# vwxyzjn/cleanrl

Hardware: AMD Instinct MI355X
Metric: env-steps/sec (SPS) PPO Breakout num_envs=1024 @1/2/4/8 MI355X; GAE HBM GB/s (higher is better)
Workload: dtype f32

## Files before the change

cleanrl_amd/build.py:

```python
from __future__ import annotations

import os
import subprocess
import sys
from concurrent.futures import ThreadPoolExecutor

CSRC = os.path.join(os.path.dirname(os.path.abspath(__file__)), "csrc")
LIB = os.path.join(CSRC, "libmi355ppo.so")
SOURCES = ["api.hip", "gae.hip", "distributions.hip", "loss.hip", "obs.hip", "optim.hip", "conv.hip", "convw.hip", "conv1q.hip", "conv1p.hip", "gemmz.hip", "gemmg.hip", "gemmh.hip", "convr.hip", "convrb.hip", "convu.hip", "fcw.hip", "heads.hip", "mlp.hip", "synth_env.hip", "dpcomm.hip", "lstm.hip", "trxl_attn.hip", "impala.hip", "pqn.hip", "pqn_lstm.hip", "offpolicy.hip", "sac.hip", "dqn.hip", "dqn_atari.hip", "rainbow.hip", "rainbow_twins.hip", "sac_atari.hip", "sac_atari_twins.hip", "qdagger.hip", "rnd.hip", "ppg.hip", "ppg_twins.hip", "host_twins.hip"]
HEADERS = ["common.h", "catrow.h", "ppo_rows.h", "lstm_rows.h", "trxl_rows.h", "impala_rows.h", "pqn_rows.h", "pqn_lstm_rows.h", "offpolicy_rows.h", "offpolicy_wg.h", "qhead_wg.h", "sac_rows.h", "dqn_rows.h", "dqn_atari_rows.h", "rainbow_rows.h", "sac_atari_rows.h", "qdagger_rows.h", "rnd_rows.h", "ppg_rows.h", "bf16split.h", "f16split.h", "convr_geom.h", "convrb_geom.h", os.path.join("..", "..", "include", "mi355ppo.h")]
HIPCC = os.environ.get("HIPCC", "/opt/rocm/bin/hipcc")
FLAGS = ["--offload-arch=gfx950", "-O3", "-std=c++20", "-ffp-contract=off", "-fPIC", "-fvisibility=hidden", "-Wall", "-Wno-unused-function"]
EXTRA_FLAGS = {"conv.hip": ["-mllvm", "-pragma-unroll-threshold=1000000"], "gemmz.hip": ["-fno-slp-vectorize"], "gemmg.hip": ["-fno-slp-vectorize"], "gemmh.hip": ["-fno-slp-vectorize", "-mllvm", "-pragma-unroll-threshold=1000000"], "convr.hip": ["-fno-slp-vectorize", "-mllvm", "-pragma-unroll-threshold=1000000"], "convrb.hip": ["-fno-slp-vectorize", "-mllvm", "-pragma-unroll-threshold=1000000"], "convu.hip": ["-fno-slp-vectorize", "-mllvm", "-pragma-unroll-threshold=1000000"], "fcw.hip": ["-fno-slp-vectorize"], "convw.hip": ["-fno-slp-vectorize"], "lstm.hip": ["-fno-slp-vectorize"], "pqn_lstm.hip": ["-fno-slp-vectorize"]}


def _stale(target: str, deps: list[str]) -> bool:
    if not os.path.exists(target):
        return True
    t = os.path.getmtime(target)
    return any(os.path.getmtime(d) > t for d in deps)


def _run(cmd: list[str]) -> None:
    r = subprocess.run(cmd, cwd=CSRC, capture_output=True, text=True)
    if r.returncode != 0:
        raise RuntimeError("command failed: %s\n%s\n%s" % (" ".join(cmd), r.stdout, r.stderr))


def build(force: bool = False, verbose: bool = True) -> str:
    hdrs = [os.path.join(CSRC, h) for h in HEADERS]
    objs, jobs = [], []
    for src in SOURCES:
        obj = os.path.join(CSRC, src.replace(".hip", ".o"))
        objs.append(obj)
        if force or _stale(obj, [os.path.join(CSRC, src)] + hdrs):
            jobs.append([HIPCC] + FLAGS + EXTRA_FLAGS.get(src, []) + ["-c", src, "-o", obj])
    if jobs:
        if verbose:
            print(f"[cleanrl_amd.build] compiling {len(jobs)} HIP source(s) for gfx950", file=sys.stderr)
        with ThreadPoolExecutor(max_workers=min(len(jobs), os.cpu_count() or 1)) as ex:
            list(ex.map(_run, jobs))
    if force or jobs or _stale(LIB, objs):
        _run([HIPCC, "--offload-arch=gfx950", "-shared", "-o", LIB] + objs)
        if verbose:
            print(f"[cleanrl_amd.build] linked {LIB}", file=sys.stderr)
    return LIB


def build_tools(verbose: bool = True) -> str:
    root = os.path.dirname(os.path.dirname(CSRC))
    src = os.path.join(root, "tools", "conv_traffic.cpp")
    exe = os.path.join(root, "tools", "conv_traffic")
    if _stale(exe, [src, LIB, os.path.join(root, "include", "mi355ppo.h")]):
        _run([HIPCC, "--offload-arch=gfx950", "-O2", "-I" + os.path.join(root, "include"), src, "-o", exe, "-L" + CSRC,
              "-lmi355ppo", "-Wl,-rpath,$ORIGIN/../cleanrl_amd/csrc"])
        if verbose:
            print(f"[cleanrl_amd.build] built {exe}", file=sys.stderr)
    fsrc, fexe = os.path.join(root, "tools", "mfma_floor.cpp"), os.path.join(root, "tools", "mfma_floor")
    if os.path.exists(fsrc) and _stale(fexe, [fsrc]):
        _run([HIPCC, "--offload-arch=gfx950", "-O3", fsrc, "-o", fexe])
        if verbose:
            print(f"[cleanrl_amd.build] built {fexe}", file=sys.stderr)
    psrc, pexe = os.path.join(root, "tools", "hbm_probe.cpp"), os.path.join(root, "tools", "hbm_probe")
    if os.path.exists(psrc) and _stale(pexe, [psrc]):
        _run([HIPCC, "--offload-arch=gfx950", "-O3", psrc, "-o", pexe])
        if verbose:
            print(f"[cleanrl_amd.build] built {pexe}", file=sys.stderr)
    dsrc, dexe = os.path.join(root, "tools", "mfma_denorm.cpp"), os.path.join(root, "tools", "mfma_denorm")
    if os.path.exists(dsrc) and _stale(dexe, [dsrc]):
        _run([HIPCC, "--offload-arch=gfx950", "-O2", "-Wno-unused-result", dsrc, "-o", dexe])
        if verbose:
            print(f"[cleanrl_amd.build] built {dexe}", file=sys.stderr)
    return exe


if __name__ == "__main__":
    build(force="--force" in sys.argv)
    build_tools()
```

cleanrl_amd/csrc/common.h:

```cpp
#pragma once
#include <hip/hip_runtime.h>
#include <stdint.h>
#include <stdio.h>
#include <stdarg.h>
#include <stdlib.h>

#include "../../include/mi355ppo.h"

#define MI355_WAVE 64
#ifndef MI355_AUX_WGRAD_LD
#define MI355_AUX_WGRAD_LD 2
#endif
#ifndef MI355_AUX_STREAM_LD
#define MI355_AUX_STREAM_LD 0
#endif
#ifndef MI355_AUX_STREAM_ST
#define MI355_AUX_STREAM_ST 0
#endif
#define MI355_HD __host__ __device__ __forceinline__

namespace mi355ppo {

void set_error(const char* fmt, ...);

int conv1p_launch(const unsigned char* src, const int64_t* inds, const float* dz, float* part_w, float* part_b, int images, int grid,
                  hipStream_t s, const unsigned* dz_amax, float* partial_scale);
bool convw_applies(int64_t images, int layer, bool f16 = false);
int convw_parts(int64_t images, int layer);
int convw_launch(const float* src, const float* dz, float* part_w, float* part_b, int64_t images, int layer, int* nparts, hipStream_t s,
                 const unsigned* dz_amax = nullptr, const unsigned* src_amax = nullptr);

bool convr_on(long long images, long long min_images);
int convr_fwd3(const char* fn, const float* src, unsigned src_bytes, const void* pack, const float* bias, float* dst, unsigned dst_bytes, unsigned* bits,
               long long images, const unsigned* src_amax, unsigned* dst_amax, hipStream_t st);
int convr_fwd2(const char* fn, const float* src, unsigned src_bytes, const void* pack, const float* bias, float* dst, unsigned dst_bytes, unsigned* bits,
               long long images, const unsigned* src_amax, unsigned* dst_amax, hipStream_t st);
int convr_dgrad3(const char* fn, const float* dz, unsigned dz_bytes, const void* pack, const unsigned* bits, float* dsrc, unsigned dsrc_bytes,
                 long long images, const unsigned* dz_amax, unsigned* dsrc_amax, hipStream_t st);
int convr_dgrad2(const char* fn, const float* dz, unsigned dz_bytes, const void* pack, const unsigned* bits, float* dsrc, unsigned dsrc_bytes,
                 long long images, const unsigned* dz_amax, unsigned* dsrc_amax, hipStream_t st);
#ifndef MI355_RING_DMA
#define MI355_RING_DMA 1
#endif
#ifndef MI355_RB_MIN_IMAGES
#define MI355_RB_MIN_IMAGES 3072
#endif
bool convrb_takes(long long images);
int convrb_dgrad2(const char* fn, const float* dz, unsigned dz_bytes, const void* pack, const unsigned* bits, float* dsrc, unsigned dsrc_bytes,
                  long long images, const unsigned* dz_amax, unsigned* dsrc_amax, hipStream_t st);
int convu_max_parts();
bool convu_takes(int64_t images, int layer);
int convu_launch(const float* src, const float* dz, float* part_w, float* part_b, int64_t images, int layer, int* nparts, hipStream_t s,
                 const unsigned* dz_amax, const unsigned* src_amax);
int convu1_launch(const unsigned char* frames, const int64_t* inds, const float* dz, float* part_w, float* part_b, int64_t images, int* nparts,
                  hipStream_t s, const unsigned* dz_amax);
bool gemmg_on(long long rows, long long min_rows);
int gemmg_launch(const char* fn, int epi, const float* A, int lda, const void* pack, const float* bias, const unsigned* bits, float* C, int M, int N,
                 int K, const unsigned* a_amax, unsigned* c_amax, hipStream_t s);
bool gemmh_takes(int M, int N, int K, int lddz);
int gemmh_slabs();
int gemmh_launch(const float* dz, int lddz, const float* a, float* part, int M, int N, int K, const unsigned* dz_amax, const unsigned* a_amax, hipStream_t s);
int z_fc_raw_launch(const char* fn, const float* a, int lda, const void* pack, int M, int N, int K, void* ws, size_t ws_bytes, int* splits,
                    hipStream_t stream, const unsigned* a_amax = nullptr);

inline hipStream_t as_stream(void* s) { return reinterpret_cast<hipStream_t>(s); }

inline int bf16_term_pairs() {
    static const int n = [] {
        const char* e = getenv("MI355PPO_BF16_PAIRS");
        return (e && e[0] == '9') ? 9 : 6;
    }();
    return n;
}

inline bool kernel_switch(const char* name, long long size, long long default_min) {
    const char* e = getenv(name);
    if (!e || !e[0]) return size >= default_min;
    if (e[0] == '0' && !e[1]) return false;
    if (e[0] == 'm' && e[1] == 'i' && e[2] == 'n' && e[3] == ':') return size >= atoll(e + 4);
    return size >= default_min;
}

inline bool aligned(const void* p, size_t a) { return (reinterpret_cast<uintptr_t>(p) % a) == 0; }

inline int check_launch(const char* what) {
    hipError_t e = hipGetLastError();
    if (e != hipSuccess) {
        set_error("%s: %s", what, hipGetErrorString(e));
        return MI355PPO_EHIP;
    }
    return MI355PPO_OK;
}

#define MI355_REQUIRE(cond, code, ...)          \
    do {                                        \
        if (!(cond)) {                          \
            ::mi355ppo::set_error(__VA_ARGS__); \
            return (code);                      \
        }                                       \
    } while (0)

#ifdef __HIPCC__

MI355_HD uint32_t mulhi_u32(uint32_t a, uint32_t b) {
#if defined(__HIP_DEVICE_COMPILE__)
    return __umulhi(a, b);
#else
    return (uint32_t)(((uint64_t)a * (uint64_t)b) >> 32);
#endif
}

struct Philox {
    uint32_t k0, k1;
    MI355_HD Philox(uint64_t seed) : k0((uint32_t)seed), k1((uint32_t)(seed >> 32)) {}
    MI355_HD uint4 operator()(uint64_t ctr_lo, uint64_t ctr_hi) const {
        uint32_t c0 = (uint32_t)ctr_lo, c1 = (uint32_t)(ctr_lo >> 32), c2 = (uint32_t)ctr_hi, c3 = (uint32_t)(ctr_hi >> 32);
        uint32_t a = k0, b = k1;
#pragma unroll
        for (int r = 0; r < 10; ++r) {
            const uint32_t hi0 = mulhi_u32(0xD2511F53u, c0), lo0 = 0xD2511F53u * c0;
            const uint32_t hi1 = mulhi_u32(0xCD9E8D57u, c2), lo1 = 0xCD9E8D57u * c2;
            const uint32_t n0 = hi1 ^ c1 ^ a, n1 = lo1, n2 = hi0 ^ c3 ^ b, n3 = lo0;
            c0 = n0; c1 = n1; c2 = n2; c3 = n3;
            a += 0x9E3779B9u; b += 0xBB67AE85u;
        }
        return make_uint4(c0, c1, c2, c3);
    }
};

MI355_HD float u32_to_unit_open(uint32_t x) {
    return ((float)(x >> 9) + 0.5f) * (1.0f / 8388608.0f);
}


__device__ __forceinline__ float wave_sum(float v) {
#pragma unroll
    for (int off = 32; off > 0; off >>= 1) v += __shfl_xor(v, off, MI355_WAVE);
    return v;
}
__device__ __forceinline__ double wave_sum(double v) {
#pragma unroll
    for (int off = 32; off > 0; off >>= 1) v += __shfl_xor(v, off, MI355_WAVE);
    return v;
}

template <int NWAVES>
__device__ __forceinline__ double block_sum(double v, double* lds) {
    v = wave_sum(v);
    const int lane = threadIdx.x & 63, wave = threadIdx.x >> 6;
    if (lane == 0) lds[wave] = v;
    __syncthreads();
    double r = 0.0;
    if (threadIdx.x == 0) {
#pragma unroll
        for (int w = 0; w < NWAVES; ++w) r += lds[w];
    }
    __syncthreads();
    return r;
}

#endif
}
```

cleanrl_amd/csrc/gemmz.hip:

```cpp
#include "common.h"
#include "conv1q_pack.h"
#include "bf16split.h"
#include "f16split.h"
#include <type_traits>

#pragma clang fp contract(off)

namespace mi355ppo {

typedef float z_f32x16 __attribute__((ext_vector_type(16)));

__device__ __forceinline__ int z_writelane(int w, unsigned x, int l) {
    asm("s_nop 1\n\tv_writelane_b32 %0, %1, %2" : "+v"(w) : "s"(x), "i"(l));
    return w;
}

enum { Z_BIAS_RELU = 0, Z_MASK = 1, Z_MASK_CLS4 = 2, Z_MASKB = 3, Z_MASKB_CLS4 = 4, Z_BIAS_RELU_BITS = 5, Z_RAW = 6 };

__device__ __forceinline__ float z_keep_where(float x, unsigned lo, unsigned hi) {
    const unsigned long long m = ((unsigned long long)hi << 32) | lo;
    float r;
    asm("s_nop 1\n\tv_cndmask_b32_e64 %0, 0, %1, %2" : "=v"(r) : "v"(x), "s"(m));
    return r;
}
// ... 954 lines not shown
}

__global__ __launch_bounds__(256) void zsplit_reduce_kernel(const float4* __restrict__ part, int splits, size_t slab4, const float* __restrict__ bias,
                                                            int n4, float4* __restrict__ h, size_t total4) {
    const size_t i = (size_t)blockIdx.x * 256 + threadIdx.x;
    if (i >= total4) return;
    float4 acc = part[i];
    for (int z = 1; z < splits; ++z) {
        const float4 p = part[(size_t)z * slab4 + i];
        acc.x += p.x; acc.y += p.y; acc.z += p.z; acc.w += p.w;
    }
    const float* const b = bias + 4 * (i % (size_t)n4);
    acc.x += b[0]; acc.y += b[1]; acc.z += b[2]; acc.w += b[3];
    h[i] = make_float4(acc.x > 0.0f ? acc.x : 0.0f, acc.y > 0.0f ? acc.y : 0.0f, acc.z > 0.0f ? acc.z : 0.0f, acc.w > 0.0f ? acc.w : 0.0f);
}

static int zsplit_steps_per(int M, int N, int K) {
    const long long tiles = (long long)((M + 63) / 64) * ((N + 63) / 64);
    const int total = K / 16;
    int target = 2 * M;
    if (target < 256) target = 256;
    if (target > 1024) target = 1024;
    long long want = (target + tiles - 1) / tiles;
    if (want < 1) want = 1;
    int per = (int)((total + want - 1) / want);
    if (per < 4) per = 4;
    if (per > total) per = total;
    return per;
}

extern "C" MI355PPO_API size_t mi355ppo_fc_fwd_workspace_bytes(int M, int N, int K) {
    constexpr int below = 8192;
    if (M <= 0 || N <= 0 || K <= 0 || K % 16 || M >= below) return 0;
    const int per = zsplit_steps_per(M, N, K), splits = (K / 16 + per - 1) / per;
    return splits > 1 ? (size_t)splits * (size_t)M * (size_t)N * sizeof(float) : 0;
}

static bool fc_g_takes(int M, int N, int K, bool dgrad) {
    return M > 0 && N > 0 && N % 32 == 0 && K >= 128 && K % 64 == 0 && gemmg_on(M, dgrad ? 1024 : 16384);
}
extern "C" MI355PPO_API int mi355ppo_fc_packed_kernel_f16x2(int M, int N, int K, int dgrad) { return fc_g_takes(M, N, K, dgrad != 0) ? 'G' : 'Z'; }

static int fc_fwd_impl(const char* fn, const float* a, int lda, const void* pack, const float* bias, float* h, int M, int N, int K,
                       const unsigned* a_amax, unsigned* h_amax, void* stream) {
    int rc = zgemm_check(fn, a, pack, h, M, N, K, lda, N);
    if (rc) return rc;
    MI355_REQUIRE(bias && aligned(bias, 4), MI355PPO_EINVAL, "%s: bias missing or misaligned", fn);
    ZArgs za = zargs(a, (long long)M * lda * 4, lda, pack, bias, nullptr, h, (long long)M * N * 4, N, M, N, K);
    za.a_amax = a_amax; za.c_amax = h_amax;
    if (a_amax && fc_g_takes(M, N, K, false)) {
        rc = gemmg_launch(fn, 0, a, lda, pack, bias, nullptr, h, M, N, K, a_amax, h_amax, as_stream(stream));
        if (rc <= 0) return rc;
    }
    if (M < 16384) return z_launch<ZRowsLinear, 2, 2, 4, Z_BIAS_RELU, true, 2>(za, as_stream(stream), fn);
    return z_launch<ZRowsLinear, 2, 4, 4, Z_BIAS_RELU, true>(za, as_stream(stream), fn);
}

extern "C" MI355PPO_API int mi355ppo_fc_fwd_relu_packed_f32(const float* a, int lda, const void* pack, const float* bias, float* h,
                                                            int M, int N, int K, void* stream) {
    return fc_fwd_impl("mi355ppo_fc_fwd_relu_packed_f32", a, lda, pack, bias, h, M, N, K, nullptr, nullptr, stream);
}

static int fc_fwd_ws_impl(const char* fn, const float* a, int lda, const void* pack, const float* bias, float* h, int M, int N, int K, void* ws,
                          size_t ws_bytes, const unsigned* a_amax, unsigned* h_amax, void* stream) {
    const size_t need = mi355ppo_fc_fwd_workspace_bytes(M, N, K);
    if (need == 0 || !ws || N % 4) return fc_fwd_impl(fn, a, lda, pack, bias, h, M, N, K, a_amax, h_amax, stream);
    MI355_REQUIRE(!h_amax, MI355PPO_EINVAL, "%s: the K-split forward (M=%d) does not record h's maximum (no consumer splits h: pass null)", fn, M);
    int rc = zgemm_check(fn, a, pack, h, M, N, K, lda, N);
    if (rc) return rc;
    MI355_REQUIRE(bias && aligned(bias, 4) && aligned(h, 16) && aligned(ws, 16), MI355PPO_EINVAL, "%s: bias missing, or h / workspace not 16-byte aligned", fn);
    MI355_REQUIRE(ws_bytes >= need, MI355PPO_EINVAL, "%s: workspace of %zu bytes, %zu needed (mi355ppo_fc_fwd_workspace_bytes)", fn, ws_bytes, need);
    ZArgs za = zargs(a, (long long)M * lda * 4, lda, pack, bias, nullptr, static_cast<float*>(ws), (long long)M * N * 4, N, M, N, K);
    za.a_amax = a_amax;
    za.steps_per = zsplit_steps_per(M, N, K);
    const int splits = (K / 16 + za.steps_per - 1) / za.steps_per;
    rc = z_launch<ZRowsLinear, 2, 2, 4, Z_RAW, true, 2>(za, as_stream(stream), fn);
    if (rc) return rc;
    const size_t total4 = (size_t)M * N / 4;
    hipLaunchKernelGGL(zsplit_reduce_kernel, dim3((unsigned)((total4 + 255) / 256)), dim3(256), 0, as_stream(stream),
                       static_cast<const float4*>(ws), splits, total4, bias, N / 4, reinterpret_cast<float4*>(h), total4);
    return check_launch(fn);
}

extern "C" MI355PPO_API int mi355ppo_fc_fwd_relu_packed_ws_f32(const float* a, int lda, const void* pack, const float* bias, float* h,
                                                               int M, int N, int K, void* ws, size_t ws_bytes, void* stream) {
    return fc_fwd_ws_impl("mi355ppo_fc_fwd_relu_packed_ws_f32", a, lda, pack, bias, h, M, N, K, ws, ws_bytes, nullptr, nullptr, stream);
}

namespace mi355ppo {
int z_fc_raw_launch(const char* fn, const float* a, int lda, const void* pack, int M, int N, int K, void* ws, size_t ws_bytes, int* splits,
                    hipStream_t stream, const unsigned* a_amax) {
    const size_t need = mi355ppo_fc_fwd_workspace_bytes(M, N, K);
    MI355_REQUIRE(need > 0 && N % 4 == 0, MI355PPO_EINVAL, "%s: M=%d rows need no K split (use the unfused entry points from 8,192 rows on)", fn, M);
    int rc = zgemm_check(fn, a, pack, static_cast<const float*>(ws), M, N, K, lda, N);
    if (rc) return rc;
    MI355_REQUIRE(ws && aligned(ws, 16) && ws_bytes >= need, MI355PPO_EWORKSPACE, "%s: workspace of %zu bytes, %zu needed (mi355ppo_fc_fwd_workspace_bytes)",
                  fn, ws ? ws_bytes : (size_t)0, need);
    ZArgs za = zargs(a, (long long)M * lda * 4, lda, pack, nullptr, nullptr, static_cast<float*>(ws), (long long)M * N * 4, N, M, N, K);
    za.a_amax = a_amax;
    za.steps_per = zsplit_steps_per(M, N, K);
    *splits = (K / 16 + za.steps_per - 1) / za.steps_per;
    return z_launch<ZRowsLinear, 2, 2, 4, Z_RAW, true, 2>(za, stream, fn);
}
}

static int fc_dgrad_impl(const char* fn, const float* dz, int lddz, const void* pack, const float* act_in, const unsigned* bits, float* da,
                         int M, int N, int K, void* stream, const unsigned* dz_amax = nullptr, unsigned* da_amax = nullptr) {
    int rc = zgemm_check(fn, dz, pack, da, M, N, K, lddz, N);
    if (rc) return rc;
    ZArgs za = zargs(dz, (long long)M * lddz * 4, lddz, pack, nullptr, act_in, da, (long long)M * N * 4, N, M, N, K);
    za.a_amax = dz_amax; za.c_amax = da_amax;
    za.super_rows = 4;
    if (bits) {
        MI355_REQUIRE(N % 32 == 0 && aligned(bits, 4) && aligned(da, 128), MI355PPO_EINVAL, "%s: bit masks need N %% 32 == 0 (N=%d) and da on a 128-byte boundary", fn, N);
        za.bits_in = bits;
        if (dz_amax && fc_g_takes(M, N, K, true)) {
            rc = gemmg_launch(fn, 1, dz, lddz, pack, nullptr, bits, da, M, N, K, dz_amax, da_amax, as_stream(stream));
            if (rc <= 0) return rc;
        }
        return z_launch<ZRowsLinear, 2, 4, 4, Z_MASKB, false>(za, as_stream(stream), fn);
    }
    MI355_REQUIRE(act_in && aligned(act_in, 4) && act_in != da, MI355PPO_EINVAL, "%s: act_in missing, misaligned or aliased with da", fn);
    return z_launch<ZRowsLinear, 2, 4, 4, Z_MASK, false>(za, as_stream(stream), fn);
}

extern "C" MI355PPO_API int mi355ppo_fc_dgrad_mask_packed_f32(const float* dz, int lddz, const void* pack, const float* act_in, float* da,
                                                              int M, int N, int K, void* stream) {
    return fc_dgrad_impl("mi355ppo_fc_dgrad_mask_packed_f32", dz, lddz, pack, act_in, nullptr, da, M, N, K, stream);
}

extern "C" MI355PPO_API int mi355ppo_fc_dgrad_maskbits_packed_f32(const float* dz, int lddz, const void* pack, const uint32_t* mask_bits,
                                                                  float* da, int M, int N, int K, void* stream) {
    const char* fn = "mi355ppo_fc_dgrad_maskbits_packed_f32";
    MI355_REQUIRE(mask_bits, MI355PPO_EINVAL, "%s: null pointer", fn);
    return fc_dgrad_impl(fn, dz, lddz, pack, nullptr, mask_bits, da, M, N, K, stream);
}

static bool conv_r_takes(long long images, int layer, bool dgrad) {
    return convr_on(images, dgrad && layer == 2 ? 512 : 1);
}

static int conv_fwd_packed_impl(const char* fn, const float* src, const void* pack, const float* bias, float* dst, unsigned* bits,
                                int64_t images, int layer, void* stream, const unsigned* src_amax = nullptr, unsigned* dst_amax = nullptr) {
    MI355_REQUIRE(src && pack && bias && dst, MI355PPO_EINVAL, "%s: null pointer", fn);
    MI355_REQUIRE(layer == 2 || layer == 3, MI355PPO_EINVAL, "%s: layer=%d must be 2 or 3", fn, layer);
    MI355_REQUIRE(images > 0, MI355PPO_EINVAL, "%s: images=%lld must be positive", fn, (long long)images);
    MI355_REQUIRE(aligned(src, 16) && aligned(pack, 16) && aligned(dst, 128) && aligned(bias, 4) && aligned(bits, 4), MI355PPO_EALIGN,
                  "%s: src / pack must be 16-byte aligned, dst 128-byte aligned", fn);
    const long long srcb = (long long)images * (layer == 2 ? 20 * 20 * 32 : 9 * 9 * 64) * 4;
    MI355_REQUIRE(srcb < (1LL << 32) - 8192, MI355PPO_EINVAL, "%s: the source (%lld bytes) must stay below 4 GiB (32-bit buffer offsets)", fn, srcb);
    hipStream_t st = as_stream(stream);
    const bool small = !bits && images < 768;
    if (layer == 2) {
        if (src_amax && conv_r_takes(images, 2, false))
            return convr_fwd2(fn, src, (unsigned)srcb, pack, bias, dst, (unsigned)((long long)images * 81 * 64 * 4), bits, images, src_amax, dst_amax, st);
        ZArgs za = zargs(src, srcb, 0, pack, bias, nullptr, dst, (long long)images * 81 * 64 * 4, 64, (long long)images * 81, 64, ZConv2::K);
        za.bits_out = bits;
        za.a_amax = src_amax; za.c_amax = dst_amax;
        if (small) return z_launch<ZConv2, 1, 2, 4, Z_BIAS_RELU, false, 2>(za, st, fn);
        if (bits) return z_blds(images) ? z_launch<ZConv2, 2, 2, 4, Z_BIAS_RELU_BITS, false, 2, true>(za, st, fn) : z_launch<ZConv2, 2, 2, 4, Z_BIAS_RELU_BITS, false, 2>(za, st, fn);
        return z_blds(images) ? z_launch<ZConv2, 2, 2, 4, Z_BIAS_RELU, false, 2, true>(za, st, fn) : z_launch<ZConv2, 2, 2, 4, Z_BIAS_RELU, false, 2>(za, st, fn);
    }
    if (src_amax && conv_r_takes(images, 3, false))
        return convr_fwd3(fn, src, (unsigned)srcb, pack, bias, dst, (unsigned)((long long)images * 49 * 64 * 4), bits, images, src_amax, dst_amax, st);
    ZArgs za = zargs(src, srcb, 0, pack, bias, nullptr, dst, (long long)images * 49 * 64 * 4, 64, (long long)images * 49, 64, ZConv3::K);
    za.bits_out = bits;
    za.a_amax = src_amax; za.c_amax = dst_amax;
    if (small) return z_launch<ZConv3, 1, 2, 4, Z_BIAS_RELU, false, 2>(za, st, fn);
    if (bits) return z_blds(images) ? z_launch<ZConv3, 2, 2, 4, Z_BIAS_RELU_BITS, false, 2, true>(za, st, fn) : z_launch<ZConv3, 2, 2, 4, Z_BIAS_RELU_BITS, false, 2>(za, st, fn);
    return z_blds(images) ? z_launch<ZConv3, 2, 2, 4, Z_BIAS_RELU, false, 2, true>(za, st, fn) : z_launch<ZConv3, 2, 2, 4, Z_BIAS_RELU, false, 2>(za, st, fn);
}

extern "C" MI355PPO_API int mi355ppo_cnn_conv_fwd_packed_f32(const float* src, const void* pack, const float* bias, float* dst,
                                                             int64_t images, int layer, void* stream) {
    return conv_fwd_packed_impl("mi355ppo_cnn_conv_fwd_packed_f32", src, pack, bias, dst, nullptr, images, layer, stream);
}

extern "C" MI355PPO_API int mi355ppo_cnn_conv_fwd_packed_bits_f32(const float* src, const void* pack, const float* bias, float* dst,
                                                                  uint32_t* mask_bits, int64_t images, int layer, void* stream) {
    const char* fn = "mi355ppo_cnn_conv_fwd_packed_bits_f32";
    MI355_REQUIRE(mask_bits, MI355PPO_EINVAL, "%s: null pointer", fn);
    return conv_fwd_packed_impl(fn, src, pack, bias, dst, mask_bits, images, layer, stream);
}

static int conv_dgrad_packed_impl(const char* fn, const float* dz, const void* pack, const float* act_in, const unsigned* bits, float* dsrc,
                                  int64_t images, int layer, void* stream, const unsigned* dz_amax = nullptr, unsigned* dsrc_amax = nullptr) {
    MI355_REQUIRE(dz && pack && (act_in || bits) && dsrc, MI355PPO_EINVAL, "%s: null pointer", fn);
    MI355_REQUIRE(layer == 2 || layer == 3, MI355PPO_EINVAL, "%s: layer=%d must be 2 or 3", fn, layer);
    MI355_REQUIRE(images > 0, MI355PPO_EINVAL, "%s: images=%lld must be positive", fn, (long long)images);
    MI355_REQUIRE(aligned(dz, 16) && aligned(pack, 16) && aligned(dsrc, 128) && aligned(act_in, 16) && aligned(bits, 4), MI355PPO_EALIGN,
                  "%s: dz / pack / act_in must be 16-byte aligned, dsrc 128-byte aligned", fn);
    MI355_REQUIRE(act_in != dsrc, MI355PPO_EINVAL, "%s: act_in must not alias dsrc", fn);
    const long long srcb = (long long)images * (layer == 2 ? 9 * 9 * 64 : 7 * 7 * 64) * 4;
    const long long dstb = (long long)images * (layer == 2 ? 20 * 20 * 32 : 9 * 9 * 64) * 4;
    MI355_REQUIRE(srcb < (1LL << 32) - 8192 && dstb < (1LL << 32) - 8192, MI355PPO_EINVAL,
                  "%s: dz (%lld bytes) and dsrc (%lld bytes) must stay below 4 GiB (32-bit buffer offsets)", fn, srcb, dstb);
    hipStream_t st = as_stream(stream);
    if (layer == 3) {
        if (dz_amax && bits && conv_r_takes(images, 3, true)) return convr_dgrad3(fn, dz, (unsigned)srcb, pack, bits, dsrc, (unsigned)dstb, images, dz_amax, dsrc_amax, st);
        ZArgs za = zargs(dz, srcb, 0, pack, nullptr, act_in, dsrc, (long long)images * 81 * 64 * 4, 64, (long long)images * 81, 64, ZDgrad3::K, images);
        za.bits_in = bits;
        za.a_amax = dz_amax; za.c_amax = dsrc_amax;
        if (bits) return z_blds(images) ? z_launch<ZDgrad3, 2, 2, 4, Z_MASKB, false, 2, true>(za, st, fn) : z_launch<ZDgrad3, 2, 2, 4, Z_MASKB, false, 2>(za, st, fn);
        return z_blds(images) ? z_launch<ZDgrad3, 2, 2, 4, Z_MASK, false, 2, true>(za, st, fn) : z_launch<ZDgrad3, 2, 2, 4, Z_MASK, false, 2>(za, st, fn);
    }
    if (dz_amax && bits && conv_r_takes(images, 2, true)) return convr_dgrad2(fn, dz, (unsigned)srcb, pack, bits, dsrc, (unsigned)dstb, images, dz_amax, dsrc_amax, st);
    ZArgs za = zargs(dz, srcb, 0, pack, nullptr, act_in, dsrc, (long long)images * 400 * 32 * 4, 0, (long long)images * 100, 128, ZDgrad2::K, images);
    za.bits_in = bits;
    za.a_amax = dz_amax; za.c_amax = dsrc_amax;
    if (bits) return z_blds(images) ? z_launch<ZDgrad2, 2, 2, 4, Z_MASKB_CLS4, false, 2, true>(za, st, fn) : z_launch<ZDgrad2, 2, 2, 4, Z_MASKB_CLS4, false, 2>(za, st, fn);
    return z_blds(images) ? z_launch<ZDgrad2, 2, 2, 4, Z_MASK_CLS4, false, 2, true>(za, st, fn) : z_launch<ZDgrad2, 2, 2, 4, Z_MASK_CLS4, false, 2>(za, st, fn);
}

extern "C" MI355PPO_API int mi355ppo_cnn_conv_dgrad_packed_f32(const float* dz, const void* pack, const float* act_in, float* dsrc,
                                                               int64_t images, int layer, void* stream) {
    const char* fn = "mi355ppo_cnn_conv_dgrad_packed_f32";
    MI355_REQUIRE(act_in, MI355PPO_EINVAL, "%s: null pointer", fn);
    return conv_dgrad_packed_impl(fn, dz, pack, act_in, nullptr, dsrc, images, layer, stream);
}

extern "C" MI355PPO_API int mi355ppo_cnn_conv_dgrad_packed_bits_f32(const float* dz, const void* pack, const uint32_t* mask_bits, float* dsrc,
                                                                    int64_t images, int layer, void* stream) {
    const char* fn = "mi355ppo_cnn_conv_dgrad_packed_bits_f32";
    MI355_REQUIRE(mask_bits, MI355PPO_EINVAL, "%s: null pointer", fn);
    return conv_dgrad_packed_impl(fn, dz, pack, nullptr, mask_bits, dsrc, images, layer, stream);
}

extern "C" MI355PPO_API int mi355ppo_cnn_conv_packed_kernel_f16x2(int64_t images, int layer, int dgrad) {
    if (!(images > 0 && (layer == 2 || layer == 3) && conv_r_takes(images, layer, dgrad != 0))) return 'Z';
    return (layer == 2 && dgrad != 0 && convrb_takes(images)) ? 'B' : 'R';
}

extern "C" MI355PPO_API size_t mi355ppo_fc_pack_f16x2_bytes(int N, int K) {
    if (N <= 0 || K <= 0 || K % 16) return 0;
    return (size_t)kF16PackHeader + (size_t)(K / 16) * (size_t)((N + 31) / 32) * 2048;
}

extern "C" MI355PPO_API int mi355ppo_absmax_f32(const float* x, int64_t n, uint32_t* amax, void* stream) {
    const char* fn = "mi355ppo_absmax_f32";
    MI355_REQUIRE(x && amax, MI355PPO_EINVAL, "%s: null pointer", fn);
    MI355_REQUIRE(n > 0, MI355PPO_EINVAL, "%s: n=%lld must be positive", fn, (long long)n);
    MI355_REQUIRE(aligned(x, 4) && aligned(amax, 64), MI355PPO_EALIGN, "%s: the amax record must be 64-byte aligned", fn);
    ZAbsmax3 m;
    m.x[0] = x; m.n[0] = n; m.x[1] = m.x[2] = x; m.n[1] = m.n[2] = 0;
    long long blocks = (n / 4 + 255) / 256;
    if (blocks < 1) blocks = 1;
    if (blocks > 2048) blocks = 2048;
    hipLaunchKernelGGL(zabsmax_kernel, dim3((unsigned)blocks), dim3(256), 0, as_stream(stream), m, amax, (int)blocks);
    return check_launch(fn);
}

extern "C" MI355PPO_API int mi355ppo_fc_pack_f16x2_f32(const float* B, int ldb, int N, int K, const uint32_t* b_amax, void* pack, void* stream) {
    const char* fn = "mi355ppo_fc_pack_f16x2_f32";
    MI355_REQUIRE(B && pack && b_amax, MI355PPO_EINVAL, "%s: null pointer", fn);
    MI355_REQUIRE(N > 0 && K > 0 && K % 16 == 0 && ldb >= K, MI355PPO_EINVAL, "%s: N=%d K=%d ldb=%d (K a positive multiple of 16, ldb >= K)", fn, N, K, ldb);
    MI355_REQUIRE(aligned(B, 4) && aligned(pack, 16) && aligned(b_amax, 64), MI355PPO_EALIGN, "%s: misaligned pointer (pack: 16 bytes, record: 64)", fn);
    const long long total = (long long)(K / 16) * ((N + 31) / 32) * 512;
    hipLaunchKernelGGL(zpack_h_kernel, dim3((unsigned)((total + 255) / 256)), dim3(256), 0, as_stream(stream), B, ldb, N, K, b_amax,
                       static_cast<unsigned char*>(pack));
    return check_launch(fn);
}

extern "C" MI355PPO_API int mi355ppo_fc_fwd_relu_packed_f16x2_f32(const float* a, int lda, const void* pack, const float* bias, float* h, int M,
                                                                  int N, int K, void* ws, size_t ws_bytes, const uint32_t* a_amax,
                                                                  uint32_t* h_amax, void* stream) {
    const char* fn = "mi355ppo_fc_fwd_relu_packed_f16x2_f32";
    MI355_REQUIRE(a_amax && aligned(a_amax, 64) && aligned(h_amax, 64), MI355PPO_EINVAL, "%s: a's amax record missing, or a record not 64-byte aligned", fn);
    return fc_fwd_ws_impl(fn, a, lda, pack, bias, h, M, N, K, ws, ws_bytes, a_amax, h_amax, stream);
}

extern "C" MI355PPO_API int mi355ppo_fc_dgrad_packed_f16x2_f32(const float* dz, int lddz, const void* pack, const float* act_in,
                                                               const uint32_t* mask_bits, float* da, int M, int N, int K, const uint32_t* dz_amax,
                                                               uint32_t* da_amax, void* stream) {
    const char* fn = "mi355ppo_fc_dgrad_packed_f16x2_f32";
    MI355_REQUIRE(dz_amax && aligned(dz_amax, 64) && aligned(da_amax, 64), MI355PPO_EINVAL, "%s: dz's amax record missing, or a record not 64-byte aligned", fn);
    MI355_REQUIRE(act_in || mask_bits, MI355PPO_EINVAL, "%s: neither act_in nor mask_bits", fn);
    return fc_dgrad_impl(fn, dz, lddz, pack, mask_bits ? nullptr : act_in, mask_bits, da, M, N, K, stream, dz_amax, da_amax);
}

extern "C" MI355PPO_API int mi355ppo_cnn_conv_fwd_packed_f16x2_f32(const float* src, const void* pack, const float* bias, float* dst,
                                                                   uint32_t* mask_bits, int64_t images, int layer, const uint32_t* src_amax,
                                                                   uint32_t* dst_amax, void* stream) {
    const char* fn = "mi355ppo_cnn_conv_fwd_packed_f16x2_f32";
    MI355_REQUIRE(src_amax && aligned(src_amax, 64) && aligned(dst_amax, 64), MI355PPO_EINVAL, "%s: src's amax record missing, or a record not 64-byte aligned", fn);
    return conv_fwd_packed_impl(fn, src, pack, bias, dst, mask_bits, images, layer, stream, src_amax, dst_amax);
}

extern "C" MI355PPO_API int mi355ppo_cnn_conv_dgrad_packed_f16x2_f32(const float* dz, const void* pack, const float* act_in,
                                                                     const uint32_t* mask_bits, float* dsrc, int64_t images, int layer,
                                                                     const uint32_t* dz_amax, uint32_t* dsrc_amax, void* stream) {
    const char* fn = "mi355ppo_cnn_conv_dgrad_packed_f16x2_f32";
    MI355_REQUIRE(dz_amax && aligned(dz_amax, 64) && aligned(dsrc_amax, 64), MI355PPO_EINVAL, "%s: dz's amax record missing, or a record not 64-byte aligned", fn);
    return conv_dgrad_packed_impl(fn, dz, pack, mask_bits ? nullptr : act_in, mask_bits, dsrc, images, layer, stream, dz_amax, dsrc_amax);
}
```

Baseline: 1.339 million.

## Add persistent stride-class conv2 forward kernel with pipelined f16 weight ring

Adds a new persistent forward kernel for conv layer 2 (20x20x32 -> 9x9x64, 4x4 stride 2). It decomposes the input into four stride-parity classes staged in LDS as split-f16 hi/lo records, and streams weights through a double-buffered DMA ring while the next group's activations are prefetched. The aim is to overlap global loads with MFMA work and cut redundant im2col-style traffic on the existing convr path. The cost is a large amount of hand-scheduled code with waitcnt/barrier logic that could be fragile. It is selected by default for batches of at least 512 images when the amax path is in use.

```diff
diff --git a/cleanrl_amd/build.py b/cleanrl_amd/build.py
--- a/cleanrl_amd/build.py
+++ b/cleanrl_amd/build.py
@@ -7,11 +7,11 @@
 
 CSRC = os.path.join(os.path.dirname(os.path.abspath(__file__)), "csrc")
 LIB = os.path.join(CSRC, "libmi355ppo.so")
-SOURCES = ["api.hip", "gae.hip", "distributions.hip", "loss.hip", "obs.hip", "optim.hip", "conv.hip", "convw.hip", "conv1q.hip", "conv1p.hip", "gemmz.hip", "gemmg.hip", "gemmh.hip", "convr.hip", "convrb.hip", "convu.hip", "fcw.hip", "heads.hip", "mlp.hip", "synth_env.hip", "dpcomm.hip", "lstm.hip", "trxl_attn.hip", "impala.hip", "pqn.hip", "pqn_lstm.hip", "offpolicy.hip", "sac.hip", "dqn.hip", "dqn_atari.hip", "rainbow.hip", "rainbow_twins.hip", "sac_atari.hip", "sac_atari_twins.hip", "qdagger.hip", "rnd.hip", "ppg.hip", "ppg_twins.hip", "host_twins.hip"]
-HEADERS = ["common.h", "catrow.h", "ppo_rows.h", "lstm_rows.h", "trxl_rows.h", "impala_rows.h", "pqn_rows.h", "pqn_lstm_rows.h", "offpolicy_rows.h", "offpolicy_wg.h", "qhead_wg.h", "sac_rows.h", "dqn_rows.h", "dqn_atari_rows.h", "rainbow_rows.h", "sac_atari_rows.h", "qdagger_rows.h", "rnd_rows.h", "ppg_rows.h", "bf16split.h", "f16split.h", "convr_geom.h", "convrb_geom.h", os.path.join("..", "..", "include", "mi355ppo.h")]
+SOURCES = ["api.hip", "gae.hip", "distributions.hip", "loss.hip", "obs.hip", "optim.hip", "conv.hip", "convw.hip", "conv1q.hip", "conv1p.hip", "gemmz.hip", "gemmg.hip", "gemmh.hip", "convr.hip", "convrb.hip", "convrs.hip", "convu.hip", "fcw.hip", "heads.hip", "mlp.hip", "synth_env.hip", "dpcomm.hip", "lstm.hip", "trxl_attn.hip", "impala.hip", "pqn.hip", "pqn_lstm.hip", "offpolicy.hip", "sac.hip", "dqn.hip", "dqn_atari.hip", "rainbow.hip", "rainbow_twins.hip", "sac_atari.hip", "sac_atari_twins.hip", "qdagger.hip", "rnd.hip", "ppg.hip", "ppg_twins.hip", "host_twins.hip"]
+HEADERS = ["common.h", "catrow.h", "ppo_rows.h", "lstm_rows.h", "trxl_rows.h", "impala_rows.h", "pqn_rows.h", "pqn_lstm_rows.h", "offpolicy_rows.h", "offpolicy_wg.h", "qhead_wg.h", "sac_rows.h", "dqn_rows.h", "dqn_atari_rows.h", "rainbow_rows.h", "sac_atari_rows.h", "qdagger_rows.h", "rnd_rows.h", "ppg_rows.h", "bf16split.h", "f16split.h", "convr_geom.h", "convrb_geom.h", "convrs_geom.h", os.path.join("..", "..", "include", "mi355ppo.h")]
 HIPCC = os.environ.get("HIPCC", "/opt/rocm/bin/hipcc")
 FLAGS = ["--offload-arch=gfx950", "-O3", "-std=c++20", "-ffp-contract=off", "-fPIC", "-fvisibility=hidden", "-Wall", "-Wno-unused-function"]
-EXTRA_FLAGS = {"conv.hip": ["-mllvm", "-pragma-unroll-threshold=1000000"], "gemmz.hip": ["-fno-slp-vectorize"], "gemmg.hip": ["-fno-slp-vectorize"], "gemmh.hip": ["-fno-slp-vectorize", "-mllvm", "-pragma-unroll-threshold=1000000"], "convr.hip": ["-fno-slp-vectorize", "-mllvm", "-pragma-unroll-threshold=1000000"], "convrb.hip": ["-fno-slp-vectorize", "-mllvm", "-pragma-unroll-threshold=1000000"], "convu.hip": ["-fno-slp-vectorize", "-mllvm", "-pragma-unroll-threshold=1000000"], "fcw.hip": ["-fno-slp-vectorize"], "convw.hip": ["-fno-slp-vectorize"], "lstm.hip": ["-fno-slp-vectorize"], "pqn_lstm.hip": ["-fno-slp-vectorize"]}
+EXTRA_FLAGS = {"conv.hip": ["-mllvm", "-pragma-unroll-threshold=1000000"], "gemmz.hip": ["-fno-slp-vectorize"], "gemmg.hip": ["-fno-slp-vectorize"], "gemmh.hip": ["-fno-slp-vectorize", "-mllvm", "-pragma-unroll-threshold=1000000"], "convr.hip": ["-fno-slp-vectorize", "-mllvm", "-pragma-unroll-threshold=1000000"], "convrb.hip": ["-fno-slp-vectorize", "-mllvm", "-pragma-unroll-threshold=1000000"], "convrs.hip": ["-fno-slp-vectorize", "-mllvm", "-pragma-unroll-threshold=1000000"], "convu.hip": ["-fno-slp-vectorize", "-mllvm", "-pragma-unroll-threshold=1000000"], "fcw.hip": ["-fno-slp-vectorize"], "convw.hip": ["-fno-slp-vectorize"], "lstm.hip": ["-fno-slp-vectorize"], "pqn_lstm.hip": ["-fno-slp-vectorize"]}
 
 
 def _stale(target: str, deps: list[str]) -> bool:
diff --git a/cleanrl_amd/csrc/common.h b/cleanrl_amd/csrc/common.h
--- a/cleanrl_amd/csrc/common.h
+++ b/cleanrl_amd/csrc/common.h
@@ -48,6 +48,12 @@
 bool convrb_takes(long long images);
 int convrb_dgrad2(const char* fn, const float* dz, unsigned dz_bytes, const void* pack, const unsigned* bits, float* dsrc, unsigned dsrc_bytes,
                   long long images, const unsigned* dz_amax, unsigned* dsrc_amax, hipStream_t st);
+#ifndef MI355_RS_MIN_IMAGES
+#define MI355_RS_MIN_IMAGES 512
+#endif
+bool convrs_takes(long long images);
+int convrs_fwd2(const char* fn, const float* src, unsigned src_bytes, const void* pack, const float* bias, float* dst, unsigned dst_bytes, unsigned* bits,
+                long long images, const unsigned* src_amax, unsigned* dst_amax, hipStream_t st);
 int convu_max_parts();
 bool convu_takes(int64_t images, int layer);
 int convu_launch(const float* src, const float* dz, float* part_w, float* part_b, int64_t images, int layer, int* nparts, hipStream_t s,
diff --git a/cleanrl_amd/csrc/convrs.hip b/cleanrl_amd/csrc/convrs.hip
--- /dev/null
+++ b/cleanrl_amd/csrc/convrs.hip
@@ -0,0 +1,267 @@
+#include "common.h"
+#include "f16split.h"
+#include "convrs_geom.h"
+
+#pragma clang fp contract(off)
+
+namespace mi355ppo {
+
+typedef float rs_f32x16 __attribute__((ext_vector_type(16)));
+
+constexpr unsigned kRSOob = 0xFFFFF000u;
+constexpr int kRSRsrcWord3 = 0x00020000;
+constexpr int kRSWaitVm0 = 0x0F70;
+
+__device__ __forceinline__ int rs_writelane(int w, unsigned x, int l) {
+    asm("s_nop 1\n\tv_writelane_b32 %0, %1, %2" : "+v"(w) : "s"(x), "i"(l));
+    return w;
+}
+
+__device__ __forceinline__ void rs_dma16(__amdgpu_buffer_rsrc_t rsrc, unsigned char* dst, unsigned voff, int soff) {
+    __builtin_amdgcn_raw_ptr_buffer_load_lds(rsrc, (__attribute__((address_space(3))) void*)dst, 16, voff, soff, 0, 0);
+}
+
+__device__ __forceinline__ void rs_put16(unsigned addr, unsigned long long hi, unsigned long long lo) {
+    asm volatile("ds_write2_b64 %0, %1, %2 offset1:8" : : "v"(addr), "v"(hi), "v"(lo) : "memory");
+}
+
+struct RSArgs {
+    const float* A;
+    unsigned a_bytes;
+    const unsigned char* pack;
+    const float* bias;
+    unsigned* bits_out;
+    float* C;
+    unsigned c_bytes;
+    long long images;
+    int groups;
+    const unsigned* a_amax;
+    unsigned* c_amax;
+};
+
+constexpr int rs_dma_younger(int slot) {
+    using RG = RSGeom;
+    int n = 0;
+    for (int r = 0; r < RG::NI; ++r) {
+        const int w = RG::round_step(r), lo = (slot * RG::SS) % RG::PSTEPS;
+        n += (w >= lo && w < lo + RG::SS - 1) ? 1 : 0;
+    }
+    return n;
+}
+
+template <bool BITS>
+__global__ __launch_bounds__(RSGeom::THREADS) __attribute__((amdgpu_waves_per_eu(2, 2))) void rs_kernel(RSArgs a) {
+    using RG = RSGeom;
+    constexpr int NT = RG::NT, NW = RG::NW, NI = RG::NI, THREADS = RG::THREADS, SS = RG::SS, NSLOT = RG::KSTEPS / SS, PSTEPS = RG::PSTEPS;
+    constexpr int kPieces = SS * NT * 2;
+    constexpr int kShare = kPieces / NW;
+    static_assert(kPieces % NW == 0 && NSLOT % 2 == 0, "whole pieces per wave; the next group's slot 0 goes to buffer 0 while the last slot is read from buffer 1");
+    __shared__ __attribute__((aligned(16))) unsigned char lds[RG::LDSB];
+    unsigned char* const ring = lds + RG::ABYTES;
+    const int tid = threadIdx.x, lane = tid & 63, wave = __builtin_amdgcn_readfirstlane(tid >> 6);
+    const int li = lane & 31, lh = lane >> 5;
+
+    const int ea = f16_scale_exp(amax_load(a.a_amax, lane));
+    const int eb = f16_scale_exp(*reinterpret_cast<const unsigned*>(a.pack));
+    const float sa = f16_pow2(ea), un = f16_unscale(ea, eb);
+
+    constexpr RRowTable<RG> table{};
+    auto row_pixel = [&](int slot, int& gi, int& gy, int& gx) __attribute__((always_inline)) {
+        const int rc = table.src[slot];
+        gi = rc / RG::OP;
+        const int pp = rc - gi * RG::OP;
+        gy = pp / RG::OW; gx = pp - gy * RG::OW;
+    };
+    constexpr unsigned kGroupC = RG::G * RG::OP * 32 * NT * 4;
+    static_assert(kGroupC < 65536, "two row offsets per register");
+    const unsigned char* win;
+    unsigned roff[8], rword;
+    {
+        int gi, gy, gx;
+        row_pixel(wave * 32 + li, gi, gy, gx);
+        win = lds + (gi * RG::IP + RG::pidx(gy, gx)) * RG::PIX + 16 * lh;
+        rword = (unsigned)((gi * RG::OP + gy * RG::OW + gx) * (32 * NT)) * 4u;
+#pragma unroll
+        for (int e = 0; e < 16; ++e) {
+            row_pixel(wave * 32 + (e & 3) + 8 * (e >> 2) + 4 * lh, gi, gy, gx);
+            const unsigned o = (unsigned)((gi * RG::OP + gy * RG::OW + gx) * (32 * NT)) * 4u + 4u * (unsigned)li;
+            roff[e >> 1] = (e & 1) ? (roff[e >> 1] | (o << 16)) : o;
+        }
+    }
+    const unsigned char* const ring_r = ring + 16 * lane;
+
+    unsigned usrc[NI], udst[NI];
+#pragma unroll
+    for (int r = 0; r < NI; ++r) {
+        const int u = r * THREADS + tid;
+        const int c4 = u % RG::UPP, j = (u / RG::UPP) % RG::CW, i = (u / (RG::UPP * RG::CW)) % RG::CH, img = u / (RG::UPP * RG::CW * RG::CH);
+        const bool ok = u < RG::CUNITS;
+        usrc[r] = ok ? (unsigned)(img * RG::IMG_SRC + (2 * i * RG::IW + 2 * j) * (RG::IC * 4) + c4 * 16) : kRSOob;
+        udst[r] = ok ? (unsigned)((img * RG::IP + i * RG::RP + j) * RG::PIX + c4 * 8) : (unsigned)(RG::SPARE * RG::PIX + c4 * 8);
+    }
+    auto rsrc_a_of = [&](int g) __attribute__((always_inline)) {
+        const bool ok = g < a.groups;
+        const unsigned gb = (unsigned)g * (unsigned)RG::GROUP_SRC;
+        return __builtin_amdgcn_make_buffer_rsrc(reinterpret_cast<unsigned char*>(const_cast<float*>(a.A)) + (ok ? gb : 0u), 0, ok ? (int)(a.a_bytes - gb) : 0, kRSRsrcWord3);
+    };
+    const unsigned lds_base = (unsigned)(uintptr_t)(__attribute__((address_space(3))) unsigned char*)lds;
+    static_assert(RG::LO == 64, "rs_put16: the lo half one ds_write2_b64 stride (8 x 8 bytes) behind the hi half");
+    s_u32x4 pre[NI];
+    auto get = [&](const __amdgpu_buffer_rsrc_t ra, int cls, int r) __attribute__((always_inline)) {
+        pre[r] = __builtin_bit_cast(s_u32x4, __builtin_amdgcn_raw_buffer_load_b128(ra, usrc[r] + (unsigned)(((cls >> 1) * RG::IW + (cls & 1)) * (RG::IC * 4)), 0, MI355_AUX_STREAM_LD));
+    };
+    auto put = [&](int buf, int r) __attribute__((always_inline)) {
+        unsigned hi[2], lo[2];
+        f16_split4(pre[r], sa, hi, lo);
+        rs_put16(lds_base + (unsigned)(buf * RG::BUFB) + udst[r], ((unsigned long long)hi[1] << 32) | hi[0], ((unsigned long long)lo[1] << 32) | lo[0]);
+    };
+
+    auto rsrc_c_of = [&](unsigned gbase) __attribute__((always_inline)) {
+        return __builtin_amdgcn_make_buffer_rsrc(reinterpret_cast<unsigned char*>(a.C) + gbase, 0, (int)(a.c_bytes - gbase), kRSRsrcWord3);
+    };
+    const __amdgpu_buffer_rsrc_t rsrc_b = __builtin_amdgcn_make_buffer_rsrc(BITS ? a.bits_out : nullptr, 0, BITS ? (int)(a.c_bytes >> 5) : 0, kRSRsrcWord3);
+    float bj[NT];
+#pragma unroll
+    for (int j = 0; j < NT; ++j) bj[j] = a.bias[32 * j + li];
+    float cmax = 0.0f;
+
+    const __amdgpu_buffer_rsrc_t rsrc_p = __builtin_amdgcn_make_buffer_rsrc(const_cast<unsigned char*>(a.pack), 0, kF16PackHeader + RG::KSTEPS * RG::STEPB, kRSRsrcWord3);
+    auto dma_slot = [&](int slot) __attribute__((always_inline)) {
+#pragma unroll
+        for (int u = 0; u < kShare; ++u) {
+            const int x = wave * kShare + u, h = x / (NT * 2), jt = x - h * (NT * 2);
+            rs_dma16(rsrc_p, ring + (slot & 1) * RG::SLOTB + x * 1024, 16u * (unsigned)lane, kF16PackHeader + r_kstep<RG>(SS * (slot % NSLOT) + h) * RG::STEPB + jt * 1024);
+        }
+    };
+    auto dma_wait = [&](int slot) __attribute__((always_inline)) {
+        const int n = rs_dma_younger(slot);
+#define RS_VMCNT_CASE(k) if (n == k) asm volatile("s_waitcnt vmcnt(" #k ")" ::: "memory");
+        RS_VMCNT_CASE(0) RS_VMCNT_CASE(1) RS_VMCNT_CASE(2) RS_VMCNT_CASE(3) RS_VMCNT_CASE(4)
+#undef RS_VMCNT_CASE
+        static_assert(RG::NI <= 5, "at most NI - 1 rounds behind a slot's pieces");
+    };
+    auto ring_barrier = [&]() __attribute__((always_inline)) {
+        asm volatile("s_waitcnt lgkmcnt(0)" ::: "memory");
+        __builtin_amdgcn_s_barrier();
+    };
+
+    rs_f32x16 acc[NT];
+    int wv = 0;
+    s_u32x4 pa[2][2], wb[2][NT][2];
+    auto read_a = [&](int par, int v) __attribute__((always_inline)) {
+        const int off = (rs_class(v) & 1) * RG::BUFB + rs_tapoff(r_kstep<RG>(v));
+        pa[par][0] = *reinterpret_cast<const s_u32x4*>(win + off);
+        pa[par][1] = *reinterpret_cast<const s_u32x4*>(win + off + RG::LO);
+    };
+    auto read_b = [&](int par, int v) __attribute__((always_inline)) {
+        const int buf = (v / SS) & 1, h = v % SS;
+#pragma unroll
+        for (int j = 0; j < NT; ++j)
+#pragma unroll
+            for (int t = 0; t < 2; ++t) wb[par][j][t] = *reinterpret_cast<const s_u32x4*>(ring_r + buf * RG::SLOTB + ((h * NT + j) * 2 + t) * 1024);
+    };
+    auto epi_elem = [&](int j, int e, unsigned gbase, const __amdgpu_buffer_rsrc_t rc) __attribute__((always_inline)) {
+        asm volatile("" : "+v"(roff[e >> 1]));
+        const unsigned rpk = roff[e >> 1];
+        const unsigned ro = ((e & 1) ? rpk >> 16 : rpk & 0xffffu) + (unsigned)(128 * j);
+        float v = __builtin_fmaf(acc[j][e], un, bj[j]);
+        v = v < 0.0f ? 0.0f : v;
+        cmax = __builtin_fmaxf(cmax, __builtin_fabsf(v));
+        __builtin_amdgcn_raw_buffer_store_b32(__float_as_uint(v), rc, ro, 0, MI355_AUX_STREAM_ST);
+        if constexpr (BITS) {
+            if (e == 0) wv = 0;
+            const unsigned long long bal = __builtin_amdgcn_ballot_w64(v > 0.0f);
+            wv = rs_writelane(wv, (unsigned)bal, (e & 3) + 8 * (e >> 2));
+            wv = rs_writelane(wv, (unsigned)(bal >> 32), (e & 3) + 8 * (e >> 2) + 4);
+            if (e == 15) __builtin_amdgcn_raw_buffer_store_b32((unsigned)wv, rsrc_b, lh == 0 ? (gbase + rword + (unsigned)(128 * j)) >> 5 : kRSOob, 0, 0);
+        }
+    };
+    static_assert(RG::round_step(NI - 1) < PSTEPS - 1, "a class is written before the barrier at its phase's last step");
+    auto group = [&](int grp) __attribute__((always_inline)) {
+        const unsigned gbase = (unsigned)grp * kGroupC;
+        const __amdgpu_buffer_rsrc_t ra_cur = rsrc_a_of(grp), ra_next = rsrc_a_of(grp + (int)gridDim.x);
+        ring_barrier();
+        read_a(0, 0);
+        read_b(0, 0);
+#pragma unroll
+        for (int v = 0; v < RG::KSTEPS; ++v) {
+            const int q = v & 1, slot = v / SS, h = v % SS, g = v / PSTEPS, w = v % PSTEPS;
+            if (h == SS - 1) dma_wait(slot);
+            if (v + 1 < RG::KSTEPS) {
+                if (h == SS - 1) ring_barrier();
+                read_b(q ^ 1, v + 1);
+                read_a(q ^ 1, v + 1);
+            }
+            if (h == 0) {
+                dma_slot(slot + 1);
+                __builtin_amdgcn_sched_barrier(0);
+            }
+#pragma unroll
+            for (int r = 0; r < NI; ++r)
+                if (w == RG::round_step(r)) {
+                    put((g + 1) & 1, r);
+                    get(g + 2 < RG::PHASES ? ra_cur : ra_next, (g + 2) % RG::PHASES, r);
+                }
+            __builtin_amdgcn_sched_barrier(0);
+#pragma unroll
+            for (int pi = 0; pi < 3; ++pi)
+#pragma unroll
+                for (int j = 0; j < NT; ++j) {
+                    if (v == 0 && pi == 0) {
+#pragma unroll
+                        for (int e = 0; e < 16; ++e) acc[j][e] = 0.0f;
+                    }
+                    acc[j] = __builtin_amdgcn_mfma_f32_32x32x16_f16(__builtin_bit_cast(s_f16x8, pa[q][pi == 2 ? 1 : 0]),
+                                                                    __builtin_bit_cast(s_f16x8, wb[q][j][pi == 1 ? 1 : 0]), acc[j], 0, 0, 0);
+                }
+            __builtin_amdgcn_sched_barrier(0);
+        }
+        const __amdgpu_buffer_rsrc_t rc = rsrc_c_of(gbase);
+#pragma unroll
+        for (int j = 0; j < NT; ++j)
+#pragma unroll
+            for (int e = 0; e < 16; ++e) epi_elem(j, e, gbase, rc);
+    };
+
+    int grp = blockIdx.x;
+    if (grp < a.groups) {
+        const __amdgpu_buffer_rsrc_t ra = rsrc_a_of(grp);
+#pragma unroll
+        for (int r = 0; r < NI; ++r) get(ra, 0, r);
+        dma_slot(0);
+        __builtin_amdgcn_s_waitcnt(kRSWaitVm0);
+#pragma unroll
+        for (int r = 0; r < NI; ++r) {
+            put(0, r);
+            get(ra, 1, r);
+        }
+        __builtin_amdgcn_s_waitcnt(kRSWaitVm0);
+    }
+    for (; grp < a.groups; grp += gridDim.x) group(grp);
+    if (a.c_amax) amax_commit(a.c_amax, __float_as_uint(cmax), blockIdx.x * NW + (unsigned)wave, lane);
+}
+
+bool convrs_takes(long long images) { return kernel_switch("MI355PPO_CONV_RS", images, MI355_RS_MIN_IMAGES); }
+
+int convrs_fwd2(const char* fn, const float* src, unsigned src_bytes, const void* pack, const float* bias, float* dst, unsigned dst_bytes, unsigned* bits,
+                long long images, const unsigned* src_amax, unsigned* dst_amax, hipStream_t st) {
+    RSArgs a{};
+    a.A = src; a.a_bytes = src_bytes; a.pack = static_cast<const unsigned char*>(pack); a.bias = bias; a.bits_out = bits; a.C = dst; a.c_bytes = dst_bytes;
+    a.images = images; a.a_amax = src_amax; a.c_amax = dst_amax;
+    a.groups = (int)((images + RSGeom::G - 1) / RSGeom::G);
+    static int cus = 0;
+    if (cus == 0) {
+        int dev = 0, n = 0;
+        if (hipGetDevice(&dev) != hipSuccess || hipDeviceGetAttribute(&n, hipDeviceAttributeMultiprocessorCount, dev) != hipSuccess || n <= 0) {
+            (void)hipGetLastError();
+            n = 256;
+        }
+        cus = n;
+    }
+    const int grid = a.groups < cus ? a.groups : cus;
+    if (bits) hipLaunchKernelGGL(rs_kernel<true>, dim3((unsigned)grid), dim3(RSGeom::THREADS), 0, st, a);
+    else hipLaunchKernelGGL(rs_kernel<false>, dim3((unsigned)grid), dim3(RSGeom::THREADS), 0, st, a);
+    return check_launch(fn);
+}
+
+}
diff --git a/cleanrl_amd/csrc/convrs_geom.h b/cleanrl_amd/csrc/convrs_geom.h
--- /dev/null
+++ b/cleanrl_amd/csrc/convrs_geom.h
@@ -0,0 +1,43 @@
+#pragma once
+
+#include "convr_geom.h"
+
+namespace mi355ppo {
+
+struct RSGeom {
+    static constexpr int IH = 20, IW = 20, IC = 32, KH = 4, KW = 4, S = 1, OH = 9, OW = 9, NT = 2, G = 3, NW = 8, MT = 1, ORDER = 2, SS = 4, WGS = 1;
+    static constexpr int NTW = NT, RW = NW;
+    static constexpr int PIX = 4 * IC + 16, LO = 2 * IC, C16 = IC / 16, UPP = IC / 4;
+    static constexpr int CH = IH / 2, CW = IW / 2;
+    static constexpr int RP = 10, IP = 101, IPIX = IP;
+    static constexpr int SPARE = CH * RP;
+    static constexpr int OP = OH * OW, ROWS = G * OP, SLOTS = 32 * MT * NW;
+    static constexpr int KSTEPS = KH * KW * C16, SPR = KW * C16, PHASES = 4, PSTEPS = KSTEPS / PHASES;
+    static constexpr int BUFB = G * IP * PIX, ABYTES = 2 * BUFB;
+    static constexpr int STEPB = NT * 2048, SLOTB = SS * STEPB;
+    static constexpr int LDSB = ABYTES + 2 * SLOTB;
+    static constexpr int THREADS = 64 * NW;
+    static constexpr int CUNITS = G * CH * CW * UPP, NI = (CUNITS + THREADS - 1) / THREADS;
+    static constexpr int IMG_SRC = IH * IW * IC * 4, GROUP_SRC = G * IMG_SRC;
+    static constexpr int pidx(int y, int x) { return y * RP + x; }
+    static constexpr int unit_src(int cls, int u) {
+        const int c4 = u % UPP, j = (u / UPP) % CW, i = (u / (UPP * CW)) % CH, img = u / (UPP * CW * CH);
+        return img * IMG_SRC + ((2 * i + (cls >> 1)) * IW + 2 * j + (cls & 1)) * (IC * 4) + c4 * 16;
+    }
+    static constexpr int unit_dst(int u) {
+        const int c4 = u % UPP, j = (u / UPP) % CW, i = (u / (UPP * CW)) % CH, img = u / (UPP * CW * CH);
+        return (img * IP + i * RP + j) * PIX + c4 * 8;
+    }
+    static constexpr int round_step(int r) { return r < 3 ? r : r + 1; }
+    static_assert((PIX / 16) % 2 == 1 && KSTEPS % (PHASES * SS) == 0 && PSTEPS == 2 * SS && ROWS <= SLOTS && NI == 5, "odd record pitch; whole ring slots per phase");
+    static_assert((G - 1) * IP + (CH - 1) * RP + CW <= G * IP && RP >= CW && IP >= CH * RP && SPARE < IP && (OH - 1 + 1) * RP + OW - 1 + 1 < SPARE, "class records inside the buffer");
+    static_assert(LDSB <= 160 * 1024, "LDS");
+};
+
+R_GEOM_FN int rs_class(int v) { return v / RSGeom::PSTEPS; }
+R_GEOM_FN int rs_tapoff(int ks) {
+    const int ty = ks / RSGeom::SPR, us = ks - ty * RSGeom::SPR, tx = us / RSGeom::C16, chunk = us - tx * RSGeom::C16;
+    return ((ty >> 1) * RSGeom::RP + (tx >> 1)) * RSGeom::PIX + chunk * 32;
+}
+
+}
diff --git a/cleanrl_amd/csrc/gemmz.hip b/cleanrl_amd/csrc/gemmz.hip
--- a/cleanrl_amd/csrc/gemmz.hip
+++ b/cleanrl_amd/csrc/gemmz.hip
@@ -1130,8 +1130,10 @@
     hipStream_t st = as_stream(stream);
     const bool small = !bits && images < 768;
     if (layer == 2) {
-        if (src_amax && conv_r_takes(images, 2, false))
+        if (src_amax && conv_r_takes(images, 2, false)) {
+            if (convrs_takes(images)) return convrs_fwd2(fn, src, (unsigned)srcb, pack, bias, dst, (unsigned)((long long)images * 81 * 64 * 4), bits, images, src_amax, dst_amax, st);
             return convr_fwd2(fn, src, (unsigned)srcb, pack, bias, dst, (unsigned)((long long)images * 81 * 64 * 4), bits, images, src_amax, dst_amax, st);
+        }
         ZArgs za = zargs(src, srcb, 0, pack, bias, nullptr, dst, (long long)images * 81 * 64 * 4, 64, (long long)images * 81, 64, ZConv2::K);
         za.bits_out = bits;
         za.a_amax = src_amax; za.c_amax = dst_amax;
```

After: 1.361 million (median of 6 runs). 1.6% higher.
